# lxd99/TPNet

Hardware: NVIDIA B200
Metric: temporal edges/sec (update+pairwise encode) (higher is better)
Workload: dtype f32

## Files before the change

include/tpnet_b200.h:

```cpp
#ifndef TPNET_B200_H_
#define TPNET_B200_H_

#include <stddef.h>
#include <stdint.h>

#ifdef __cplusplus
extern "C" {
#endif

#define TPN_ABI_VERSION 11

#define TPN_MAX_LAYERS 4

enum {
    TPN_OK = 0,
    TPN_ERR_INVALID_ARGUMENT = -1,
    TPN_ERR_WORKSPACE_TOO_SMALL = -2,
    TPN_ERR_LOG_FULL = -3,
    TPN_ERR_CUDA = -4,
    TPN_ERR_UNSUPPORTED = -5,
    TPN_ERR_INDEX = -6
};

typedef struct tpn_state {
// ... 28 lines not shown
#define TPN_UPDATE_WHOLE 0
#define TPN_UPDATE_PREPARE 1
#define TPN_UPDATE_APPLY 2
int tpn_update_phase(tpn_state_t* st,
                     const int64_t* src_dev, const int64_t* dst_dev, const double* t_dev, int64_t batch,
                     double t_last, float neg_lambda, const float* decay,
                     void* ws_dev, size_t ws_bytes, int32_t* err_flag_dev, void* stream, int phase);

#define TPN_DEBUG_PER_LAYER_WALK 1
#define TPN_DEBUG_SERIAL_WALK 2
#define TPN_DEBUG_SNAPSHOT_P0 4
#define TPN_DEBUG_HEAD_FFMA 8
#define TPN_DEBUG_LEGACY_FRONT 16
#define TPN_DEBUG_NO_STREAM 32
#define TPN_DEBUG_STREAM_ALL 64
int tpn_set_debug_flags(int flags);


int tpn_update_messages(tpn_state_t* st,
                        const int64_t* tgt_dev, const int64_t* src_dev, const double* t_dev, int64_t num_messages,
                        const int32_t* num_messages_dev, int64_t num_local_rows,
                        double t_last, float neg_lambda, const float* decay,
                        void* ws_dev, size_t ws_bytes, int32_t* err_flag_dev, void* stream);

int tpn_gather_blocks(const tpn_state_t* st, const int64_t* ids_dev, int64_t n, float* out_dev, void* stream);

int tpn_pairwise(const tpn_state_t* st, const int64_t* a_ids_dev, const int64_t* b_ids_dev, int64_t n,
                 const int32_t* n_dev, int apply_log_scale, float* out_dev, void* stream);

int tpn_pairwise_neighbors(const tpn_state_t* st, const int64_t* nbr_dev, const int64_t* src_dev,
                           const int64_t* dst_dev, int64_t m, int num_neighbors, int apply_log_scale,
// ... 72 lines not shown
```

tpnet_b200/_lib.py:

```python
from __future__ import annotations

import ctypes
import os
from ctypes import POINTER, c_char_p, c_double, c_float, c_int, c_int32, c_int64, c_size_t, c_void_p
from typing import Optional

_PKG = os.path.dirname(os.path.abspath(__file__))
LIB_PATH = os.path.join(_PKG, '_C', 'libtpnet_b200.so')

TPN_OK = 0
TPN_ERR_LOG_FULL = -3
TPN_ERR_UNSUPPORTED = -5
TPN_ERR_INDEX = -6
STAGE_RAW, STAGE_ID_WRAP, STAGE_ID = 0, 1, 2
TPN_MAX_LAYERS = 4
UPDATE_WHOLE, UPDATE_PREPARE, UPDATE_APPLY = 0, 1, 2
ABI_VERSION = 11

EXPORTED_SYMBOLS = (
    'tpn_version', 'tpn_error_string', 'tpn_last_cuda_error', 'tpn_device_info',
    'tpn_update_workspace_bytes', 'tpn_update', 'tpn_update_phase', 'tpn_pairwise', 'tpn_gather',
    'tpn_materialize', 'tpn_reset_epoch', 'tpn_clear_walk_layers',
    'tpn_stager_create', 'tpn_stager_destroy', 'tpn_stage',
    'tpn_update_messages', 'tpn_gather_blocks', 'tpn_set_debug_flags', 'tpn_pairwise_neighbors', 'tpn_head_forward',
    'tpn_planner_create', 'tpn_planner_destroy', 'tpn_plan', 'tpn_sampler_recent',
    'tpn_route_workspace_bytes', 'tpn_route_update', 'tpn_route_pairs', 'tpn_pull_rows', 'tpn_peer_barrier',
    'tpn_shard_new_generation', 'tpn_peer_alloc', 'tpn_peer_free', 'tpn_ipc_export', 'tpn_ipc_open', 'tpn_ipc_close',
)

SHARD_CTR_NEED, SHARD_CTR_PREV, SHARD_CTR_ERROR, SHARD_COUNTERS = 0, 1, 2, 8


class TpnState(ctypes.Structure):
    _fields_ = [
        ('data', c_void_p),
        ('num_nodes', c_int64),
        ('num_layer', c_int32),
        ('dim', c_int32),
        ('row_stride', c_int64),
# ... 45 lines not shown
    lib.tpn_device_info.restype = c_int
    lib.tpn_device_info.argtypes = [POINTER(c_int), POINTER(c_int), POINTER(c_int)]
    lib.tpn_update_workspace_bytes.restype = c_size_t
    lib.tpn_update_workspace_bytes.argtypes = [POINTER(TpnState), c_int64]
    lib.tpn_update.restype = c_int
    lib.tpn_update.argtypes = [POINTER(TpnState), c_void_p, c_void_p, c_void_p, c_int64, c_double, c_float,
                               POINTER(c_float), c_void_p, c_size_t, c_void_p, c_void_p]
    lib.tpn_update_phase.restype = c_int
    lib.tpn_update_phase.argtypes = [POINTER(TpnState), c_void_p, c_void_p, c_void_p, c_int64, c_double, c_float,
                                     POINTER(c_float), c_void_p, c_size_t, c_void_p, c_void_p, c_int]
    lib.tpn_update_messages.restype = c_int
    lib.tpn_update_messages.argtypes = [POINTER(TpnState), c_void_p, c_void_p, c_void_p, c_int64, c_void_p, c_int64,
                                        c_double, c_float, POINTER(c_float), c_void_p, c_size_t, c_void_p, c_void_p]
    lib.tpn_set_debug_flags.restype = c_int
    lib.tpn_set_debug_flags.argtypes = [c_int]
    lib.tpn_gather_blocks.restype = c_int
    lib.tpn_gather_blocks.argtypes = [POINTER(TpnState), c_void_p, c_int64, c_void_p, c_void_p]
    lib.tpn_pairwise.restype = c_int
    lib.tpn_pairwise.argtypes = [POINTER(TpnState), c_void_p, c_void_p, c_int64, c_void_p, c_int, c_void_p, c_void_p]
    lib.tpn_pairwise_neighbors.restype = c_int
    lib.tpn_pairwise_neighbors.argtypes = [POINTER(TpnState), c_void_p, c_void_p, c_void_p, c_int64, c_int, c_int,
                                           c_void_p, c_void_p]
    lib.tpn_head_forward.restype = c_int
    lib.tpn_head_forward.argtypes = [c_void_p, c_int64, c_void_p, c_int, c_int, c_void_p, c_void_p, c_void_p, c_void_p,
                                     c_void_p, c_void_p]
    lib.tpn_gather.restype = c_int
    lib.tpn_gather.argtypes = [POINTER(TpnState), c_void_p, c_int64, c_void_p, c_void_p]
    for name in ('tpn_materialize', 'tpn_reset_epoch', 'tpn_clear_walk_layers'):
        fn = getattr(lib, name)
        fn.restype = c_int
# ... 77 lines not shown
```

tpnet_b200/csrc/tpn_head_tc.cu:

```cuda
#include <cuda_fp16.h>

#include "tpn_common.cuh"

namespace tpn {

namespace {

constexpr int kF = 64;
constexpr int kHid = 256;
constexpr int kTile = 128;
constexpr int kTcThreads = 160;
constexpr uint32_t kTmemCols = 512;
constexpr uint32_t kD2Col = 256;
constexpr uint32_t kLbo = 128;
constexpr uint32_t kSbo = 1024;
constexpr uint32_t kKStepBytes = 256;

struct TcSmem {
    __half w1[2][kHid * kF];
    __half w2[2][4][kF * 64];
    __half x[2][kTile * kF];
    __half h[2][2][kTile * 64];
    float b1[kHid];
    float b2[kF];
    uint64_t x_full, d1_full, d2_full, h_full[2], h_empty[2];
    uint32_t tmem_base;
    float red[8];
    float w1_inv, w2_inv;
};

__device__ __forceinline__ int canon(int row, int k) { return (row >> 3) * 512 + (k >> 3) * 64 + (row & 7) * 8 + (k & 7); }

__device__ __forceinline__ uint64_t smem_desc(const void* p) {
    const uint32_t addr = smem_u32(p);
    uint64_t d = (uint64_t)((addr & 0x3FFFFu) >> 4);
    d |= (uint64_t)(kLbo >> 4) << 16;
    d |= (uint64_t)(kSbo >> 4) << 32;
    d |= (uint64_t)1 << 46;
    return d;
}

__device__ __forceinline__ constexpr uint32_t instr_desc(int m, int n) {
    return (1u << 4) | ((uint32_t)(n >> 3) << 17) | ((uint32_t)(m >> 4) << 24);
}
// ... 76 lines not shown
                    *reinterpret_cast<uint32_t*>(&l[2]), *reinterpret_cast<uint32_t*>(&l[3]));
}

__device__ __forceinline__ float pow2_scale(float vmax) {
    if (!(vmax > 0.f) || !(vmax < 3.0e38f)) return 1.0f;
    int e;
    (void)frexpf(vmax, &e);
    int s = 14 - e;
    s = s > 100 ? 100 : (s < -100 ? -100 : s);
    return ldexpf(1.0f, s);
}

__global__ void __launch_bounds__(kTcThreads, 1)
head_tc_kernel(const float* __restrict__ x, long long n, const float* __restrict__ w1, const float* __restrict__ b1,
               const float* __restrict__ w2, const float* __restrict__ b2, float* __restrict__ y,
               const int* __restrict__ n_dev) {
    if (n_dev != nullptr) n = min(n, (long long)max(*n_dev, 0));
    extern __shared__ __align__(128) unsigned char tc_raw[];
    TcSmem& sm = *reinterpret_cast<TcSmem*>(tc_raw);
    const int tid = threadIdx.x, warp = tid >> 5, lane = tid & 31;
    const long long ntiles = (n + kTile - 1) / kTile;

    if (tid == 0) {
        mbar_init(&sm.x_full, kTile);
        mbar_init(&sm.d1_full, 1);
        mbar_init(&sm.d2_full, 1);
        for (int i = 0; i < 2; ++i) {
            mbar_init(&sm.h_full[i], kTile);
            mbar_init(&sm.h_empty[i], 1);
        }
        asm volatile("fence.mbarrier_init.release.cluster;" ::: "memory");
// ... 58 lines not shown
    tc_fence_after();
    const uint32_t tmem = sm.tmem_base;
    const float w1_inv = sm.w1_inv, w2_inv = sm.w2_inv;

    uint32_t it = 0;
    if (warp < 4) {
        const int r = tid;
        const uint32_t lane_base = (uint32_t)(warp * 32) << 16;
        float4 xn[kF / 4];
        auto load_x = [&](long long tile) {
            const long long row = tile * kTile + r;
            const bool ok = tile < ntiles && row < n;
#pragma unroll
            for (int q = 0; q < kF / 4; ++q) xn[q] = ok ? ld4(x + row * kF + 4 * q) : make_float4(0.f, 0.f, 0.f, 0.f);
        };
        auto split_x = [&]() -> float {
            float vmax = 0.f;
#pragma unroll
            for (int q = 0; q < kF / 4; ++q)
                vmax = fmaxf(vmax, fmaxf(fmaxf(fabsf(xn[q].x), fabsf(xn[q].y)), fmaxf(fabsf(xn[q].z), fabsf(xn[q].w))));
            const float sx = pow2_scale(vmax);
#pragma unroll
            for (int k8 = 0; k8 < kF / 8; ++k8) {
                const float4 a = xn[2 * k8], b = xn[2 * k8 + 1];
                const float v[8] = {a.x * sx, a.y * sx, a.z * sx, a.w * sx, b.x * sx, b.y * sx, b.z * sx, b.w * sx};
                uint4 hi, lo;
                split8(v, hi, lo);
                *reinterpret_cast<uint4*>(&sm.x[0][canon(r, k8 * 8)]) = hi;
                *reinterpret_cast<uint4*>(&sm.x[1][canon(r, k8 * 8)]) = lo;
            }
            fence_proxy_async_smem();
            tc_fence_before();
            mbar_arrive(&sm.x_full);
            return w1_inv / sx;
        };
        long long tile = blockIdx.x;
        load_x(tile);
        float inv1 = split_x();
        load_x(tile + gridDim.x);
        for (; tile < ntiles; tile += gridDim.x, ++it) {
            const long long row = tile * kTile + r;
            const bool valid = row < n;
            mbar_wait_bounded(&sm.d1_full, it & 1u);
            tc_fence_after();
            float inv2[4];
#pragma unroll 1
            for (int c = 0; c < 4; ++c) {
                const int buf = c & 1;
                const uint32_t use = it * 2u + (uint32_t)(c >> 1);
                float d0[32], d1[32];
                tmem_ld32_nowait(tmem + lane_base + (uint32_t)(c * 64), d0);
                tmem_ld32_nowait(tmem + lane_base + (uint32_t)(c * 64 + 32), d1);
                tmem_ld_wait();
                float hmax = 0.f;
#pragma unroll
// ... 7 lines not shown
                mbar_wait_bounded(&sm.h_empty[buf], (use & 1u) ^ 1u);
#pragma unroll
                for (int k8 = 0; k8 < 8; ++k8) {
                    float v[8];
#pragma unroll
                    for (int j = 0; j < 8; ++j) v[j] = (k8 < 4 ? d0[k8 * 8 + j] : d1[(k8 - 4) * 8 + j]) * sh;
                    uint4 hi, lo;
                    split8(v, hi, lo);
                    *reinterpret_cast<uint4*>(&sm.h[buf][0][canon(r, k8 * 8)]) = hi;
                    *reinterpret_cast<uint4*>(&sm.h[buf][1][canon(r, k8 * 8)]) = lo;
                }
                fence_proxy_async_smem();
                mbar_arrive(&sm.h_full[buf]);
            }
            const float inv2_0 = inv2[0], inv2_1 = inv2[1], inv2_2 = inv2[2], inv2_3 = inv2[3];
            if (tile + gridDim.x < ntiles) {
                inv1 = split_x();
                load_x(tile + 2 * (long long)gridDim.x);
            }
            mbar_wait_bounded(&sm.d2_full, it & 1u);
            tc_fence_after();
#pragma unroll 1
            for (int half = 0; half < 2; ++half) {
                float d[32];
                {
                    float d1[32], d2[32], d3[32];
                    tmem_ld32_nowait(tmem + lane_base + kD2Col + (uint32_t)(half * 32), d);
                    tmem_ld32_nowait(tmem + lane_base + kD2Col + 64u + (uint32_t)(half * 32), d1);
                    tmem_ld32_nowait(tmem + lane_base + kD2Col + 128u + (uint32_t)(half * 32), d2);
                    tmem_ld32_nowait(tmem + lane_base + kD2Col + 192u + (uint32_t)(half * 32), d3);
                    tmem_ld_wait();
#pragma unroll
                    for (int j = 0; j < 32; ++j)
                        d[j] = (d[j] * inv2_0 + d1[j] * inv2_1) + (d2[j] * inv2_2 + d3[j] * inv2_3);
                }
                if (valid) {
#pragma unroll
                    for (int q = 0; q < 8; ++q) {
                        const int o = half * 32 + q * 4;
                        st4(y + row * kF + o, make_float4(d[q * 4] + sm.b2[o], d[q * 4 + 1] + sm.b2[o + 1],
                                                          d[q * 4 + 2] + sm.b2[o + 2], d[q * 4 + 3] + sm.b2[o + 3]));
                    }
                }
            }
            tc_fence_before();
        }
    } else if (lane == 0) {
        constexpr uint32_t idesc1 = instr_desc(kTile, kHid), idesc2 = instr_desc(kTile, kF);
        const uint64_t xa[2] = {smem_desc(sm.x[0]), smem_desc(sm.x[1])};
        const uint64_t wb[2] = {smem_desc(sm.w1[0]), smem_desc(sm.w1[1])};
        auto gemm1 = [&](uint32_t t) {
            mbar_wait_bounded(&sm.x_full, t & 1u);
            tc_fence_after();
#pragma unroll
            for (int ks = 0; ks < kF / 16; ++ks) {
                const uint64_t adv = (uint64_t)((ks * kKStepBytes) >> 4);
                mma_f16(tmem, xa[0] + adv, wb[1] + adv, idesc1, ks > 0 ? 1u : 0u);
                mma_f16(tmem, xa[1] + adv, wb[0] + adv, idesc1, 1u);
            }
#pragma unroll
            for (int ks = 0; ks < kF / 16; ++ks) {
                const uint64_t adv = (uint64_t)((ks * kKStepBytes) >> 4);
                mma_f16(tmem, xa[0] + adv, wb[0] + adv, idesc1, 1u);
            }
            mma_commit(&sm.d1_full);
        };
        long long tile = blockIdx.x;
        if (tile < ntiles) gemm1(0);
        for (; tile < ntiles; tile += gridDim.x, ++it) {
#pragma unroll 1
            for (int c = 0; c < 4; ++c) {
                const int buf = c & 1;
                const uint32_t use = it * 2u + (uint32_t)(c >> 1);
                mbar_wait_bounded(&sm.h_full[buf], use & 1u);
                tc_fence_after();
                const uint64_t ha[2] = {smem_desc(sm.h[buf][0]), smem_desc(sm.h[buf][1])};
                const uint64_t vb[2] = {smem_desc(sm.w2[0][c]), smem_desc(sm.w2[1][c])};
                const uint32_t dacc = tmem + kD2Col + (uint32_t)(c * 64);
#pragma unroll
                for (int ks = 0; ks < 4; ++ks) {
                    const uint64_t adv = (uint64_t)((ks * kKStepBytes) >> 4);
                    mma_f16(dacc, ha[0] + adv, vb[1] + adv, idesc2, ks > 0 ? 1u : 0u);
                    mma_f16(dacc, ha[1] + adv, vb[0] + adv, idesc2, 1u);
                }
#pragma unroll
                for (int ks = 0; ks < 4; ++ks) {
                    const uint64_t adv = (uint64_t)((ks * kKStepBytes) >> 4);
                    mma_f16(dacc, ha[0] + adv, vb[0] + adv, idesc2, 1u);
                }
                mma_commit(&sm.h_empty[buf]);
            }
            mma_commit(&sm.d2_full);
            if (tile + gridDim.x < ntiles) gemm1(it + 1u);
        }
    }

    tc_fence_before();
    __syncthreads();
    if (warp == 4) {
        asm volatile("tcgen05.dealloc.cta_group::1.sync.aligned.b32 %0, %1;" ::"r"(tmem), "r"(kTmemCols) : "memory");
    }
}

}

int launch_head_tensor(const float* x, long long n, const int* n_dev, const float* w1, const float* b1, const float* w2,
                       const float* b2, float* y, int dev_slot, cudaStream_t stream) {
    static bool configured_tab[kMaxDevices];
    bool& configured = configured_tab[dev_slot];
    const int smem = (int)sizeof(TcSmem);
    if (!configured) {
        const cudaError_t e = cudaFuncSetAttribute(head_tc_kernel, cudaFuncAttributeMaxDynamicSharedMemorySize, smem);
        if (e != cudaSuccess) {
            set_cuda_error(e);
            return TPN_ERR_CUDA;
        }
        configured = true;
    }
    const long long ntiles = (n + kTile - 1) / kTile;
    const int sms = device_sm_count();
    const unsigned grid = (unsigned)(ntiles < sms ? ntiles : sms);
    head_tc_kernel<<<grid, kTcThreads, smem, stream>>>(x, n, w1, b1, w2, b2, y, n_dev);
    return TPN_OK;
}

}
```

tpnet_b200/csrc/tpn_update.cu:

```cuda
#include <stdlib.h>

#include "tpn_common.cuh"

namespace tpn {

namespace {

int g_debug_flags = 0;
thread_local int g_dev_slot = 0;

constexpr int kSmallMaxMsgs = 4096;
constexpr int kRankMaxMsgs = 1024;
constexpr int kPrepThreads = 1024;
constexpr int kRadixThreads = 256;
constexpr int kRadixItems = 8;
constexpr int kRadixTile = kRadixThreads * kRadixItems;
constexpr int kRadixBins = 256;
constexpr int kRadixDirectBlocks = 16;
constexpr int kWalkThreads = 256;
constexpr int kHubMin = 64;
constexpr int kGiantMin = 2048;
constexpr int kHubConsumers = 4;
constexpr int kHubThreads = (kHubConsumers + 1) * 32;
constexpr int kHubStages = 4;
// ... 8 lines not shown
#ifndef TPN_HUB2_GIANT_FLOATS
#define TPN_HUB2_GIANT_FLOATS 16
#endif
constexpr int kHub2GiantFloats = TPN_HUB2_GIANT_FLOATS;
static_assert(kHub2GiantFloats == 8 || kHub2GiantFloats == 16 || kHub2GiantFloats == 32, "giant slices are 32, 64 or 128 bytes");
constexpr int kGiantLs = kHub2GiantFloats == 8 ? 1 : (kHub2GiantFloats == 16 ? 2 : 3);
constexpr int kGiantSpm = 16 >> kGiantLs;
constexpr int kGiantSpmMax = kGiantSpm > 4 ? kGiantSpm : 4;
constexpr int kHub2Stages = kHub2Producers + 4;
constexpr int kCtrGiant = 0, kCtrHub = 1, kCtrWork0 = 2, kCtrSmall = 6, kCtrHub2Work = 7, kCtrHub2Giant = 8;
constexpr int kCtrChunks = 9;
constexpr int kCtrStream = 10, kCtrStreamBlocks = 11, kCtrStreamProd = 12, kCtrStreamActive = 13, kCtrStreamChain = 14, kCtrStreamTicket = 15;
constexpr int kStreamSlice = kHub2GiantFloats;
constexpr int kStreamBlock = 32 * kGiantSpm;
constexpr uint32_t kNoPart = 0xffffffffu;
constexpr int kCtrSmClaim = 16;
constexpr int kCtrSlots = kCtrSmClaim + 256;
constexpr int kBarWords = 32;

struct DecayArgs {
    float c[TPN_MAX_LAYERS];
    int has_decay;
};

struct Count {
    int cap;
    const int* dev;
    __device__ __forceinline__ int get() const {
        if (dev == nullptr) return cap;
        const int v = *dev;
        return v < 0 ? 0 : (v > cap ? cap : v);
// ... 36 lines not shown
    uint32_t* sslot;
    uint32_t* slen;
    float* snap;
    uint32_t* hub_giant;
    uint32_t* hub_reg;
    uint32_t* ctr;
    uint32_t* small_heads;
    uint32_t* hub_len;
    uint32_t* hub_part;
    uint32_t* giant_cbase;
    float* partial;
    int* svst;
    float* gprod;
    uint32_t* gflag;
    uint32_t* gblk;
    bool has_snap;
    bool has_stream;
    size_t bytes;
};

inline size_t snap_bytes(size_t E, int num_layer, int64_t row_stride) {
    return sizeof(float) * E * (size_t)num_layer * (size_t)row_stride;
}

inline size_t align_up(size_t x, size_t a) { return (x + a - 1) / a * a; }

constexpr size_t kStreamMaxBytes = (size_t)4 << 30;
constexpr int kGiantSortMaxC = 2048;
inline int stream_slices(int num_layer, int64_t row_stride) {
    return num_layer * (int)((row_stride + kStreamSlice - 1) / kStreamSlice);
// ... 28 lines not shown
    const size_t hub_cap = E / kHubMin + E / kChunkMin + E / kGiantMin + 4;
    const size_t part_rows = E / kChunkMin + E / kGiantMin + 2;
    ws.hub_reg = reinterpret_cast<uint32_t*>(take(4 * hub_cap));
    ws.hub_len = reinterpret_cast<uint32_t*>(take(4 * hub_cap));
    ws.hub_part = reinterpret_cast<uint32_t*>(take(4 * hub_cap));
    ws.giant_cbase = reinterpret_cast<uint32_t*>(take(4 * (E / kGiantMin + 2)));
    ws.partial = reinterpret_cast<float*>(take(ws.has_snap ? 4 * part_rows * (size_t)num_layer * (size_t)row_stride : 16));
    ws.ctr = reinterpret_cast<uint32_t*>(take(4 * kCtrSlots));
    ws.small_heads = reinterpret_cast<uint32_t*>(take(4 * E));
    ws.svst = reinterpret_cast<int*>(take(4 * (E + 4) * (size_t)(num_layer > 1 ? num_layer - 1 : 1) + 16));
    ws.gflag = reinterpret_cast<uint32_t*>(take(4 * stream_flag_words(E)));
    ws.gblk = reinterpret_cast<uint32_t*>(take(4 * (kGiantSortMaxC + 1)));
    ws.has_stream = ws.has_snap && stream_prod_bytes(E, num_layer, row_stride) <= kStreamMaxBytes &&
                    E / kGiantMin + 2 <= (size_t)kGiantSortMaxC;
    ws.gprod = reinterpret_cast<float*>(take(ws.has_stream ? stream_prod_bytes(E, num_layer, row_stride) : 16));
    ws.bytes = off;
    return ws;
}

__device__ __forceinline__ float edge_weight(double t, float t_last_f, float neg_lambda) {
    const float diff = __fsub_rn(t_last_f, (float)t);
    const float arg = __fmul_rn(neg_lambda, diff);
    return (float)exp((double)arg);
}

struct SweepArgs {
    long long total4;
    int ds4;
};

// ... 460 lines not shown
        if (small_head) small_heads[base + __popc(mask & ((1u << lane) - 1u))] = (uint32_t)p;
    }
}

__global__ void __launch_bounds__(256) payload_kernel(PayloadArgs a) {
    payload_body(a, blockIdx.x * blockDim.x + threadIdx.x);
}

constexpr int kGiantSortMax = kGiantSortMaxC;
struct GiantSmem {
    uint32_t head_s[kGiantSortMax], len_s[kGiantSortMax], sorted_s[kGiantSortMax];
};
__device__ __forceinline__ void sort_giants_body(GiantSmem& sm, uint32_t* __restrict__ hub_giant,
                                                 const uint32_t* __restrict__ slen, uint32_t* __restrict__ ctr,
                                                 uint32_t* __restrict__ gblk, uint32_t* __restrict__ gflag, Count count,
                                                 int stream_mode) {
    const uint32_t stream_min = stream_mode == 0 ? 0u
                                : (stream_mode == 2 ? (uint32_t)kGiantMin
                                                    : max((uint32_t)kGiantMin, (uint32_t)(count.get() >> 2)));
    const int n = (int)ctr[kCtrGiant];
    if (n < 1 || n > kGiantSortMax) return;
    for (int i = threadIdx.x; i < n; i += blockDim.x) {
        sm.head_s[i] = hub_giant[i];
        sm.len_s[i] = slen[sm.head_s[i]];
    }
    __syncthreads();
    for (int i = threadIdx.x; i < n; i += blockDim.x) {
        const uint32_t li = sm.len_s[i];
        int rank = 0;
        for (int j = 0; j < n; ++j) rank += (sm.len_s[j] > li || (sm.len_s[j] == li && j < i)) ? 1 : 0;
        hub_giant[rank] = sm.head_s[i];
        sm.sorted_s[rank] = li;
    }
    __syncthreads();
    if (threadIdx.x == 0 && stream_min > 0) {
        uint32_t blocks = 0;
        int ns = 0;
        for (; ns < n && sm.sorted_s[ns] >= stream_min; ++ns) {
            gblk[ns] = blocks;
            blocks += (sm.sorted_s[ns] + (uint32_t)kStreamBlock - 1u) / (uint32_t)kStreamBlock;
        }
        gblk[ns] = blocks;
        ctr[kCtrStream] = (uint32_t)ns;
        ctr[kCtrStreamBlocks] = blocks;
        sm.head_s[0] = blocks;
    }
    __syncthreads();
    if (stream_min > 0) {
        const uint32_t blocks = sm.head_s[0];
        for (uint32_t i = threadIdx.x; i < blocks; i += blockDim.x) gflag[i] = 0;
    }
}
__global__ void __launch_bounds__(1024)
sort_giants_kernel(uint32_t* __restrict__ hub_giant, const uint32_t* __restrict__ slen, uint32_t* __restrict__ ctr,
                   uint32_t* __restrict__ gblk, uint32_t* __restrict__ gflag, Count count, int stream_mode) {
    __shared__ GiantSmem sm;
    sort_giants_body(sm, hub_giant, slen, ctr, gblk, gflag, count, stream_mode);
}

struct FrontArgs {
    PrepArgs prep;
    uint32_t *key_a, *key_b, *val_a, *val_b, *hist, *hist2, *bar;
    int passes;
};

__device__ __forceinline__ void grid_barrier(uint32_t* bar, uint32_t& target, int* err_flag) {
    __syncthreads();
    if (threadIdx.x == 0) {
        target += gridDim.x;
        __threadfence();
        atomicAdd(bar, 1u);
        uint32_t seen;
// ... 892 lines not shown
    }
}

__host__ __device__ inline size_t hub2_smem_bytes() {
    return (size_t)kHub2Stages * (32 * kHub2SlotFloats * 4 + 16) + 16;
}

template <bool LAZY, bool DIRECT>
__global__ void __launch_bounds__(kHub2Threads, 2)
walk_hub2_kernel(StateView st, const uint32_t* __restrict__ skey, const uint32_t* __restrict__ ssrc,
                 const float* __restrict__ sw, const uint32_t* __restrict__ sslot,
                 const uint32_t* __restrict__ slen, const float* __restrict__ snap,
                 const uint32_t* __restrict__ hub_giant, const uint32_t* __restrict__ hub_reg,
                 uint32_t* __restrict__ ctr, int spr_g, int slice_w_g, int spr_r, int slice_w_r, DecayArgs dnow,
                 const uint32_t* __restrict__ hub_len, const uint32_t* __restrict__ hub_part,
                 float* __restrict__ partial, int chunked, int srow0) {
    extern __shared__ __align__(128) unsigned char hub2_raw[];
    float* const ring = reinterpret_cast<float*>(hub2_raw);
    uint64_t* const full = reinterpret_cast<uint64_t*>(ring + (size_t)kHub2Stages * 32 * kHub2SlotFloats);
    uint64_t* const empty = full + kHub2Stages;
    int* const item = reinterpret_cast<int*>(empty + kHub2Stages);
    const int warp = threadIdx.x >> 5;
    const int lane = threadIdx.x & 31;
    const int L = st.num_layer;
    const int rs = (int)st.row_stride;
    if (threadIdx.x == 0) {
        for (int i = 0; i < kHub2Stages; ++i) {
            mbar_init(&full[i], 32);
            mbar_init(&empty[i], 1);
        }
        asm volatile("fence.mbarrier_init.release.cluster;" ::: "memory");
        unsigned smid;
        asm volatile("mov.u32 %0, %%smid;" : "=r"(smid));
        *item = (smid < 256u && atomicAdd(&ctr[kCtrSmClaim + smid], 1u) == 0u) ? 1 : 0;
    }
    __syncthreads();
    const bool prefer_giant = *item != 0;
    __syncthreads();
    const uint32_t n_stream = ctr[kCtrStream];
    const uint32_t n_giant = ctr[kCtrGiant] - n_stream, n_reg = ctr[kCtrHub];
    const uint32_t slices_g = (uint32_t)(L * spr_g), slices_r = (uint32_t)(L * spr_r);
    const uint32_t total_g = chunked ? 0u : n_giant * slices_g, total_r = n_reg * slices_r;
    uint32_t blk_base = 0;
    for (;;) {
        if (threadIdx.x == 0) {
            int w = -1;
            if (prefer_giant && total_g > 0) {
                const uint32_t g = atomicAdd(&ctr[kCtrHub2Giant], 1u);
                if (g < total_g) w = (int)g;
            }
            if (w == -1 && total_r > 0) {
                const uint32_t q = atomicAdd(&ctr[kCtrHub2Work], 1u);
                if (q < total_r) w = -(int)q - 2;
            }
            *item = w;
        }
        __syncthreads();
        const int work = *item;
        __syncthreads();
        if (work == -1) break;
        const bool giant = work >= 0;
        const uint32_t idx = giant ? (uint32_t)work : (uint32_t)(-(work + 2));
        const int spr = giant ? spr_g : spr_r;
        const int slice_w = giant ? slice_w_g : slice_w_r;
        const uint32_t slices = giant ? slices_g : slices_r;
        const uint32_t hub_i = idx / slices;
        const int slice = (int)(idx - hub_i * slices);
        const uint32_t hub = giant ? hub_i + n_stream : hub_i;
        const int r = slice / spr;
        const int c0 = (slice - r * spr) * slice_w;
        const int width = min(rs, c0 + slice_w) - c0;
        const int head = (int)(giant ? hub_giant[hub] : hub_reg[hub]);
        const int len = (int)(giant ? slen[head] : hub_len[hub]);
        const uint32_t part = giant ? kNoPart : hub_part[hub];
        const uint32_t key = skey[head];
        const int spm = giant ? kGiantSpm : 1;
        const int slot = giant ? kHub2GiantFloats : kHub2SlotFloats;
        const int mps = 32 * spm;
        const int nblk = (len + mps - 1) / mps;
        if (width > 0) {
            if (warp >= 1) {
                const int pw = warp - 1;
                const int nvec = width >> 2;
// ... 114 lines not shown
                                acc.y = __fadd_rn(acc.y, p.y);
                            }
                        }
                        for (; j0 < nm; ++j0) {
                            const float2 p = *reinterpret_cast<const float2*>(xs + j0 * kHub2SlotFloats);
                            acc.x = __fadd_rn(acc.x, p.x);
                            acc.y = __fadd_rn(acc.y, p.y);
                        }
                    }
                    HUB2_STAMP(b, 2);
                    __syncwarp();
                    if (lane == 0) mbar_arrive(&empty[stage]);
                    HUB2_STAMP(b, 3);
                }
                if (active) {
                    if (giant) *tptr = acc.x;
                    else *reinterpret_cast<float2*>(tptr) = acc;
                }
            }
        }
        blk_base += (width > 0) ? (uint32_t)nblk : 0u;
    }
}

template <bool LAZY>
__global__ void __launch_bounds__(256)
combine_giants_kernel(StateView st, const uint32_t* __restrict__ skey, const uint32_t* __restrict__ slen,
                      const uint32_t* __restrict__ hub_giant, const uint32_t* __restrict__ giant_cbase,
                      const uint32_t* __restrict__ ctr, const float* __restrict__ partial, int chunk) {
    const int L = st.num_layer;
    const int rs = (int)st.row_stride;
// ... 15 lines not shown
            uint32_t c = 0;
            for (; c + 4 <= nch; c += 4) {
                const float p0 = pbase[(long long)(c + 0) * span + col], p1 = pbase[(long long)(c + 1) * span + col];
                const float p2 = pbase[(long long)(c + 2) * span + col], p3 = pbase[(long long)(c + 3) * span + col];
                acc = __fadd_rn(__fadd_rn(__fadd_rn(__fadd_rn(acc, p0), p1), p2), p3);
            }
            for (; c < nch; ++c) acc = __fadd_rn(acc, pbase[(long long)c * span + col]);
            trow[col] = acc;
        }
    }
}


template <bool DIRECT>
int launch_walk_hub2(const StateView& v, const Workspace& ws, bool lazy, const DecayArgs& dnow, int chunk, int srow0,
                     cudaStream_t stream) {
    static bool configured_tab[kMaxDevices];
    bool& configured = configured_tab[g_dev_slot];
    const int smem = (int)hub2_smem_bytes();
    if (!configured) {
        cudaError_t e = cudaFuncSetAttribute(walk_hub2_kernel<false, DIRECT>, cudaFuncAttributeMaxDynamicSharedMemorySize, smem);
        if (e == cudaSuccess)
            e = cudaFuncSetAttribute(walk_hub2_kernel<true, DIRECT>, cudaFuncAttributeMaxDynamicSharedMemorySize, smem);
        if (e != cudaSuccess) {
            set_cuda_error(e);
            return TPN_ERR_CUDA;
        }
        configured = true;
    }
    const int rs = (int)v.row_stride;
    const int spr_r = (rs + kHub2SlotFloats - 1) / kHub2SlotFloats;
    const int slice_w_r = (((rs + spr_r - 1) / spr_r) + 3) & ~3;
    const int spr_g = (rs + kHub2GiantFloats - 1) / kHub2GiantFloats;
    const int slice_w_g = (((rs + spr_g - 1) / spr_g) + 3) & ~3;
    const unsigned grid = (unsigned)device_sm_count() * 2;
    const int chunked = chunk > 0 ? 1 : 0;
    if (lazy)
        walk_hub2_kernel<true, DIRECT><<<grid, kHub2Threads, smem, stream>>>(v, ws.key_a, ws.ssrc, ws.sw, ws.sslot, ws.slen,
                                                                             ws.snap, ws.hub_giant, ws.hub_reg, ws.ctr,
                                                                             spr_g, slice_w_g, spr_r, slice_w_r, dnow,
                                                                             ws.hub_len, ws.hub_part, ws.partial, chunked,
                                                                             srow0);
    else
        walk_hub2_kernel<false, DIRECT><<<grid, kHub2Threads, smem, stream>>>(v, ws.key_a, ws.ssrc, ws.sw, ws.sslot, ws.slen,
                                                                              ws.snap, ws.hub_giant, ws.hub_reg, ws.ctr,
                                                                              spr_g, slice_w_g, spr_r, slice_w_r, dnow,
                                                                              ws.hub_len, ws.hub_part, ws.partial, chunked,
                                                                              srow0);
    if (chunked) {
        const unsigned cgrid = (unsigned)device_sm_count();
        if (lazy)
            combine_giants_kernel<true><<<cgrid, 256, 0, stream>>>(v, ws.key_a, ws.slen, ws.hub_giant, ws.giant_cbase,
                                                                   ws.ctr, ws.partial, chunk);
        else
            combine_giants_kernel<false><<<cgrid, 256, 0, stream>>>(v, ws.key_a, ws.slen, ws.hub_giant, ws.giant_cbase,
                                                                    ws.ctr, ws.partial, chunk);
    }
    return TPN_OK;
}

template <bool DIRECT>
int launch_walk_stream(const StateView& v, const Workspace& ws, bool lazy, int srow0, int* err_flag_dev, cudaStream_t stream) {
    static bool configured_tab[kMaxDevices];
// ... 185 lines not shown
    const float t_last_f = (float)t_last;
    double* log_w = lazy ? st->decay_log : nullptr;
    const bool force_per_layer = (g_debug_flags & TPN_DEBUG_PER_LAYER_WALK) != 0;
    const bool snapshot_path = ws.has_snap && !(force_per_layer && !(count_dev == nullptr && E <= kSmallMaxMsgs));
    const bool small_path = count_dev == nullptr && E <= kSmallMaxMsgs;
    const bool hubs = !small_path;
    const int E4 = (E + 3) & ~3;
    const bool eager_sweep = !lazy && dargs.has_decay;
    int chunk = st->giant_chunk > 0 ? (int)st->giant_chunk : 0;
    if (chunk > 0 && chunk < kChunkMin) chunk = kChunkMin;
    if (chunk > kGiantMin) chunk = kGiantMin;
    chunk &= ~31;
    const long long sweep_total4 = st->num_nodes * (long long)L * ds4;
    const int stream_mode = (ws.has_stream && chunk == 0 && (g_debug_flags & TPN_DEBUG_NO_STREAM) == 0)
                                ? ((g_debug_flags & TPN_DEBUG_STREAM_ALL) ? 2 : 1) : 0;

    StateView view = make_view(st);
    view.epoch = new_epoch;

    const bool do_front = phase != TPN_UPDATE_APPLY;
    const bool do_rest = phase != TPN_UPDATE_PREPARE;
    const bool snap_early = lazy && !small_path;
    if (small_path) {
        if (phase == TPN_UPDATE_PREPARE) return TPN_OK;
        SweepArgs sw_args;
        sw_args.total4 = eager_sweep ? sweep_total4 : 0;
        sw_args.ds4 = ds4;
        unsigned grid = 1;
        if (eager_sweep) {
            const long long want = (sweep_total4 + kPrepThreads - 1) / kPrepThreads;
// ... 56 lines not shown
            fr.passes = passes;
            const int sms = device_sm_count();
            const unsigned grid = (unsigned)(nblk < 1 ? 1 : (nblk < sms ? nblk : sms));
            void* kargs[] = {&fr};
            if (cudaMemsetAsync(ws.bar, 0, 4 * kBarWords, stream) != cudaSuccess ||
                cudaLaunchCooperativeKernel((const void*)front_kernel, dim3(grid), dim3(kRadixThreads), kargs, 0,
                                            stream) != cudaSuccess) {
                set_cuda_error(cudaGetLastError());
                return TPN_ERR_CUDA;
            }
            const bool odd = (passes & 1) != 0;
            fa.pay.order = odd ? ws.val_b : ws.val_a;
            fa.pay.skey = odd ? ws.key_b : ws.key_a;
            payload_kernel<<<(E + 255) / 256, 256, 0, stream>>>(fa.pay);
            if (snapshot_path && chunk == 0) {
                sort_giants_kernel<<<1, 1024, 0, stream>>>(ws.hub_giant, ws.slen, ws.ctr, ws.gblk, ws.gflag, cnt, stream_mode);
            }
        } else
        {
            prep_large_kernel<<<(unsigned)((E + 255) / 256 < 2 ? 2 : (E + 255) / 256), 256, 0, stream>>>(fa.prep);
            uint32_t *kin = ws.key_a, *kout = ws.key_b, *vin = ws.val_a, *vout = ws.val_b;
            for (int p = 0; p < passes; ++p) {
                radix_hist_kernel<<<nblk, kRadixThreads, 0, stream>>>(kin, cnt, 8 * p, ws.hist);
                const int prefixed = (nblk > kRadixDirectBlocks || count_dev != nullptr) ? 1 : 0;
                if (prefixed) radix_prefix_kernel<<<kRadixBins / 8, 256, 0, stream>>>(ws.hist, cnt);
                radix_scatter_kernel<<<nblk, kRadixThreads, 0, stream>>>(kin, vin, kout, vout, cnt, 8 * p, ws.hist,
                                                                         prefixed);
                uint32_t* tk = kin; kin = kout; kout = tk;
                uint32_t* tv = vin; vin = vout; vout = tv;
            }
            fa.pay.order = vin;
            fa.pay.skey = kin;
            payload_kernel<<<(E + 255) / 256, 256, 0, stream>>>(fa.pay);
            if (snapshot_path && chunk == 0) {
                sort_giants_kernel<<<1, 1024, 0, stream>>>(ws.hub_giant, ws.slen, ws.ctr, ws.gblk, ws.gflag, cnt, stream_mode);
            }
        }
    }
    if (!small_path && do_rest && eager_sweep) {
        const long long want = (sweep_total4 + 255) / 256;
        const long long cap = (long long)device_sm_count() * 16;
        const unsigned grid = (unsigned)(want < cap ? (want < 1 ? 1 : want) : cap);
        sweep_decay_kernel<<<grid, 256, 0, stream>>>(view, dargs, sweep_total4, ds4);
    }

    const int srow0 = (g_debug_flags & TPN_DEBUG_SNAPSHOT_P0) ? 0 : 1;
    if (snapshot_path) {
        if (L - srow0 >= 1 && (snap_early ? do_front : do_rest)) {
            const unsigned grid = (unsigned)(((long long)E * 32 + 255) / 256);
            if (lazy) snapshot_kernel<true><<<grid, 256, 0, stream>>>(view, ws.key_a, cnt, ds4, ws.snap, srow0);
            else snapshot_kernel<false><<<grid, 256, 0, stream>>>(view, ws.key_a, cnt, ds4, ws.snap, srow0);
        }
        if (!do_rest) {
        } else if (hubs) {
            const bool direct = msgs.B == 0;
            SideStream* side = (g_debug_flags & TPN_DEBUG_SERIAL_WALK) ? nullptr : side_stream();
            cudaStream_t hub_stream = stream, giant_stream = stream;
            if (side != nullptr) {
                if (cudaEventRecord(side->fork, stream) == cudaSuccess &&
                    cudaStreamWaitEvent(side->stream, side->fork, 0) == cudaSuccess) {
                    hub_stream = side->stream;
                    if (stream_mode > 0 && cudaStreamWaitEvent(side->stream2, side->fork, 0) == cudaSuccess)
                        giant_stream = side->stream2;
                } else {
                    (void)cudaGetLastError();
                }
            }
            if (stream_mode > 0) {
// ... 60 lines not shown
    const size_t have = sizeof(tpn::g_hub2_timeline) / sizeof(unsigned long long);
    if (host_out == nullptr || count > have) return TPN_ERR_INVALID_ARGUMENT;
    return cudaMemcpyFromSymbol(host_out, tpn::g_hub2_timeline, count * sizeof(unsigned long long)) == cudaSuccess
               ? TPN_OK : TPN_ERR_CUDA;
}
#endif

namespace tpn {
int debug_flags() { return g_debug_flags; }
}

extern "C" int tpn_set_debug_flags(int flags) {
    const int old = tpn::g_debug_flags;
    tpn::g_debug_flags = flags;
    return old;
}

extern "C" int tpn_update(tpn_state_t* st, const int64_t* src_dev, const int64_t* dst_dev, const double* t_dev,
                          int64_t batch, double t_last, float neg_lambda, const float* decay, void* ws_dev,
                          size_t ws_bytes, int32_t* err_flag_dev, void* stream_v) {
    using namespace tpn;
    int rc = validate_state(st);
    if (rc != TPN_OK) return rc;
    if (batch < 1 || batch > ((int64_t)1 << 26) || src_dev == nullptr || dst_dev == nullptr || t_dev == nullptr ||
        ws_dev == nullptr || st->num_nodes >= (int64_t)0xffffffffll)
        return TPN_ERR_INVALID_ARGUMENT;
    DeviceScope scope(st->data);
    g_dev_slot = scope.slot();
    MsgSource msgs;
    msgs.a = reinterpret_cast<const long long*>(src_dev);
// ... 52 lines not shown
```

Before: 155.0 million.

## Precompute largest giant hubs during prepare phase; dynamic tile claiming in head kernel

During the PREPARE phase, up to two of the largest giant hubs are walked early into a workspace buffer. The APPLY phase then copies those results into state and skips them in the giant work queue, moving long-tail work earlier so it can overlap with other stages. Separately, the tensor-core head kernel now hands out tiles through a global atomic counter with per-launch claim slots instead of a fixed grid stride, for better load balance. This adds a workspace buffer, extra atomics and barriers, and a debug query function.

```diff
diff --git a/include/tpnet_b200.h b/include/tpnet_b200.h
--- a/include/tpnet_b200.h
+++ b/include/tpnet_b200.h
@@ -66,7 +66,9 @@
 #define TPN_DEBUG_LEGACY_FRONT 16
 #define TPN_DEBUG_NO_STREAM 32
 #define TPN_DEBUG_STREAM_ALL 64
+#define TPN_DEBUG_NO_EARLY_GIANTS 128
 int tpn_set_debug_flags(int flags);
+int tpn_debug_early_giants(const tpn_state_t* st, int64_t batch, const void* ws_dev, int32_t* count_out);
 
 
 int tpn_update_messages(tpn_state_t* st,
diff --git a/tpnet_b200/_lib.py b/tpnet_b200/_lib.py
--- a/tpnet_b200/_lib.py
+++ b/tpnet_b200/_lib.py
@@ -22,7 +22,7 @@
     'tpn_update_workspace_bytes', 'tpn_update', 'tpn_update_phase', 'tpn_pairwise', 'tpn_gather',
     'tpn_materialize', 'tpn_reset_epoch', 'tpn_clear_walk_layers',
     'tpn_stager_create', 'tpn_stager_destroy', 'tpn_stage',
-    'tpn_update_messages', 'tpn_gather_blocks', 'tpn_set_debug_flags', 'tpn_pairwise_neighbors', 'tpn_head_forward',
+    'tpn_update_messages', 'tpn_gather_blocks', 'tpn_set_debug_flags', 'tpn_debug_early_giants', 'tpn_pairwise_neighbors', 'tpn_head_forward',
     'tpn_planner_create', 'tpn_planner_destroy', 'tpn_plan', 'tpn_sampler_recent',
     'tpn_route_workspace_bytes', 'tpn_route_update', 'tpn_route_pairs', 'tpn_pull_rows', 'tpn_peer_barrier',
     'tpn_shard_new_generation', 'tpn_peer_alloc', 'tpn_peer_free', 'tpn_ipc_export', 'tpn_ipc_open', 'tpn_ipc_close',
@@ -98,6 +98,8 @@
                                         c_double, c_float, POINTER(c_float), c_void_p, c_size_t, c_void_p, c_void_p]
     lib.tpn_set_debug_flags.restype = c_int
     lib.tpn_set_debug_flags.argtypes = [c_int]
+    lib.tpn_debug_early_giants.restype = c_int
+    lib.tpn_debug_early_giants.argtypes = [POINTER(TpnState), c_int64, c_void_p, POINTER(c_int32)]
     lib.tpn_gather_blocks.restype = c_int
     lib.tpn_gather_blocks.argtypes = [POINTER(TpnState), c_void_p, c_int64, c_void_p, c_void_p]
     lib.tpn_pairwise.restype = c_int
diff --git a/tpnet_b200/csrc/tpn_head_tc.cu b/tpnet_b200/csrc/tpn_head_tc.cu
--- a/tpnet_b200/csrc/tpn_head_tc.cu
+++ b/tpnet_b200/csrc/tpn_head_tc.cu
@@ -24,10 +24,20 @@
     float b1[kHid];
     float b2[kF];
     uint64_t x_full, d1_full, d2_full, h_full[2], h_empty[2];
+    long long claimed;
+    uint32_t x_valid;
     uint32_t tmem_base;
     float red[8];
     float w1_inv, w2_inv;
 };
+
+constexpr int kClaimSlots = 256;
+struct TileClaim {
+    unsigned long long next;
+    unsigned int done;
+    unsigned int pad;
+};
+__device__ TileClaim g_head_claim[kClaimSlots];
 
 __device__ __forceinline__ int canon(int row, int k) { return (row >> 3) * 512 + (k >> 3) * 64 + (row & 7) * 8 + (k & 7); }
 
@@ -134,7 +144,7 @@
 __global__ void __launch_bounds__(kTcThreads, 1)
 head_tc_kernel(const float* __restrict__ x, long long n, const float* __restrict__ w1, const float* __restrict__ b1,
                const float* __restrict__ w2, const float* __restrict__ b2, float* __restrict__ y,
-               const int* __restrict__ n_dev) {
+               const int* __restrict__ n_dev, int claim_slot) {
     if (n_dev != nullptr) n = min(n, (long long)max(*n_dev, 0));
     extern __shared__ __align__(128) unsigned char tc_raw[];
     TcSmem& sm = *reinterpret_cast<TcSmem*>(tc_raw);
@@ -223,7 +233,20 @@
 #pragma unroll
             for (int q = 0; q < kF / 4; ++q) xn[q] = ok ? ld4(x + row * kF + 4 * q) : make_float4(0.f, 0.f, 0.f, 0.f);
         };
-        auto split_x = [&]() -> float {
+        TileClaim& claim = g_head_claim[claim_slot];
+        auto next_tile = [&]() -> long long {
+            if (tid == 0) sm.claimed = (long long)gridDim.x + (long long)atomicAdd(&claim.next, 1ull);
+            asm volatile("bar.sync 1, %0;" ::"n"(kTile) : "memory");
+            const long long t = sm.claimed;
+            asm volatile("bar.sync 1, %0;" ::"n"(kTile) : "memory");
+            return t;
+        };
+        auto split_x = [&](bool valid) -> float {
+            if (r == 0) sm.x_valid = valid ? 1u : 0u;
+            if (!valid) {
+                mbar_arrive(&sm.x_full);
+                return 0.f;
+            }
             float vmax = 0.f;
 #pragma unroll
             for (int q = 0; q < kF / 4; ++q)
@@ -245,9 +268,10 @@
         };
         long long tile = blockIdx.x;
         load_x(tile);
-        float inv1 = split_x();
-        load_x(tile + gridDim.x);
-        for (; tile < ntiles; tile += gridDim.x, ++it) {
+        float inv1 = split_x(tile < ntiles);
+        long long next = tile < ntiles ? next_tile() : ntiles;
+        load_x(next);
+        for (; tile < ntiles; ++it) {
             const long long row = tile * kTile + r;
             const bool valid = row < n;
             mbar_wait_bounded(&sm.d1_full, it & 1u);
@@ -285,9 +309,11 @@
                 mbar_arrive(&sm.h_full[buf]);
             }
             const float inv2_0 = inv2[0], inv2_1 = inv2[1], inv2_2 = inv2[2], inv2_3 = inv2[3];
-            if (tile + gridDim.x < ntiles) {
-                inv1 = split_x();
-                load_x(tile + 2 * (long long)gridDim.x);
+            inv1 = split_x(next < ntiles);
+            long long after = ntiles;
+            if (next < ntiles) {
+                after = next_tile();
+                load_x(after);
             }
             mbar_wait_bounded(&sm.d2_full, it & 1u);
             tc_fence_after();
@@ -315,14 +341,17 @@
                 }
             }
             tc_fence_before();
+            tile = next;
+            next = after;
         }
     } else if (lane == 0) {
         constexpr uint32_t idesc1 = instr_desc(kTile, kHid), idesc2 = instr_desc(kTile, kF);
         const uint64_t xa[2] = {smem_desc(sm.x[0]), smem_desc(sm.x[1])};
         const uint64_t wb[2] = {smem_desc(sm.w1[0]), smem_desc(sm.w1[1])};
-        auto gemm1 = [&](uint32_t t) {
+        auto gemm1 = [&](uint32_t t) -> bool {
             mbar_wait_bounded(&sm.x_full, t & 1u);
             tc_fence_after();
+            if (sm.x_valid == 0u) return false;
 #pragma unroll
             for (int ks = 0; ks < kF / 16; ++ks) {
                 const uint64_t adv = (uint64_t)((ks * kKStepBytes) >> 4);
@@ -335,10 +364,9 @@
                 mma_f16(tmem, xa[0] + adv, wb[0] + adv, idesc1, 1u);
             }
             mma_commit(&sm.d1_full);
+            return true;
         };
-        long long tile = blockIdx.x;
-        if (tile < ntiles) gemm1(0);
-        for (; tile < ntiles; tile += gridDim.x, ++it) {
+        for (bool more = gemm1(0); more; ++it) {
 #pragma unroll 1
             for (int c = 0; c < 4; ++c) {
                 const int buf = c & 1;
@@ -362,7 +390,7 @@
                 mma_commit(&sm.h_empty[buf]);
             }
             mma_commit(&sm.d2_full);
-            if (tile + gridDim.x < ntiles) gemm1(it + 1u);
+            more = gemm1(it + 1u);
         }
     }
 
@@ -370,6 +398,13 @@
     __syncthreads();
     if (warp == 4) {
         asm volatile("tcgen05.dealloc.cta_group::1.sync.aligned.b32 %0, %1;" ::"r"(tmem), "r"(kTmemCols) : "memory");
+    }
+    if (tid == 0) {
+        TileClaim& claim = g_head_claim[claim_slot];
+        if (atomicAdd(&claim.done, 1u) == gridDim.x - 1u) {
+            claim.next = 0ull;
+            claim.done = 0u;
+        }
     }
 }
 
@@ -391,7 +426,9 @@
     const long long ntiles = (n + kTile - 1) / kTile;
     const int sms = device_sm_count();
     const unsigned grid = (unsigned)(ntiles < sms ? ntiles : sms);
-    head_tc_kernel<<<grid, kTcThreads, smem, stream>>>(x, n, w1, b1, w2, b2, y, n_dev);
+    static unsigned next_slot[kMaxDevices];
+    const int slot = (int)(next_slot[dev_slot]++ % (unsigned)kClaimSlots);
+    head_tc_kernel<<<grid, kTcThreads, smem, stream>>>(x, n, w1, b1, w2, b2, y, n_dev, slot);
     return TPN_OK;
 }
 
diff --git a/tpnet_b200/csrc/tpn_update.cu b/tpnet_b200/csrc/tpn_update.cu
--- a/tpnet_b200/csrc/tpn_update.cu
+++ b/tpnet_b200/csrc/tpn_update.cu
@@ -46,7 +46,10 @@
 constexpr int kStreamSlice = kHub2GiantFloats;
 constexpr int kStreamBlock = 32 * kGiantSpm;
 constexpr uint32_t kNoPart = 0xffffffffu;
-constexpr int kCtrSmClaim = 16;
+constexpr int kCtrEarly = 16, kCtrEarlyWork = 17;
+constexpr int kEarlyMax = 2;
+constexpr int kEarlyShift = 4;
+constexpr int kCtrSmClaim = 18;
 constexpr int kCtrSlots = kCtrSmClaim + 256;
 constexpr int kBarWords = 32;
 
@@ -113,6 +116,7 @@
     float* gprod;
     uint32_t* gflag;
     uint32_t* gblk;
+    float* early;
     bool has_snap;
     bool has_stream;
     size_t bytes;
@@ -171,6 +175,7 @@
     ws.has_stream = ws.has_snap && stream_prod_bytes(E, num_layer, row_stride) <= kStreamMaxBytes &&
                     E / kGiantMin + 2 <= (size_t)kGiantSortMaxC;
     ws.gprod = reinterpret_cast<float*>(take(ws.has_stream ? stream_prod_bytes(E, num_layer, row_stride) : 16));
+    ws.early = reinterpret_cast<float*>(take(sizeof(float) * kEarlyMax * (size_t)num_layer * (size_t)row_stride));
     ws.bytes = off;
     return ws;
 }
@@ -661,10 +666,11 @@
 __device__ __forceinline__ void sort_giants_body(GiantSmem& sm, uint32_t* __restrict__ hub_giant,
                                                  const uint32_t* __restrict__ slen, uint32_t* __restrict__ ctr,
                                                  uint32_t* __restrict__ gblk, uint32_t* __restrict__ gflag, Count count,
-                                                 int stream_mode) {
+                                                 int stream_mode, int early_max) {
     const uint32_t stream_min = stream_mode == 0 ? 0u
                                 : (stream_mode == 2 ? (uint32_t)kGiantMin
                                                     : max((uint32_t)kGiantMin, (uint32_t)(count.get() >> 2)));
+    const uint32_t early_min = max((uint32_t)kGiantMin, (uint32_t)(count.get() >> kEarlyShift));
     const int n = (int)ctr[kCtrGiant];
     if (n < 1 || n > kGiantSortMax) return;
     for (int i = threadIdx.x; i < n; i += blockDim.x) {
@@ -680,17 +686,22 @@
         sm.sorted_s[rank] = li;
     }
     __syncthreads();
-    if (threadIdx.x == 0 && stream_min > 0) {
-        uint32_t blocks = 0;
+    if (threadIdx.x == 0) {
         int ns = 0;
-        for (; ns < n && sm.sorted_s[ns] >= stream_min; ++ns) {
+        if (stream_min > 0) {
+            uint32_t blocks = 0;
+            for (; ns < n && sm.sorted_s[ns] >= stream_min; ++ns) {
+                gblk[ns] = blocks;
+                blocks += (sm.sorted_s[ns] + (uint32_t)kStreamBlock - 1u) / (uint32_t)kStreamBlock;
+            }
             gblk[ns] = blocks;
-            blocks += (sm.sorted_s[ns] + (uint32_t)kStreamBlock - 1u) / (uint32_t)kStreamBlock;
-        }
-        gblk[ns] = blocks;
-        ctr[kCtrStream] = (uint32_t)ns;
-        ctr[kCtrStreamBlocks] = blocks;
-        sm.head_s[0] = blocks;
+            ctr[kCtrStream] = (uint32_t)ns;
+            ctr[kCtrStreamBlocks] = blocks;
+            sm.head_s[0] = blocks;
+        }
+        int ne = 0;
+        while (ne < early_max && ns + ne < n && sm.sorted_s[ns + ne] >= early_min) ++ne;
+        ctr[kCtrEarly] = (uint32_t)ne;
     }
     __syncthreads();
     if (stream_min > 0) {
@@ -700,9 +711,10 @@
 }
 __global__ void __launch_bounds__(1024)
 sort_giants_kernel(uint32_t* __restrict__ hub_giant, const uint32_t* __restrict__ slen, uint32_t* __restrict__ ctr,
-                   uint32_t* __restrict__ gblk, uint32_t* __restrict__ gflag, Count count, int stream_mode) {
+                   uint32_t* __restrict__ gblk, uint32_t* __restrict__ gflag, Count count, int stream_mode,
+                   int early_max) {
     __shared__ GiantSmem sm;
-    sort_giants_body(sm, hub_giant, slen, ctr, gblk, gflag, count, stream_mode);
+    sort_giants_body(sm, hub_giant, slen, ctr, gblk, gflag, count, stream_mode, early_max);
 }
 
 struct FrontArgs {
@@ -1625,7 +1637,7 @@
                  const uint32_t* __restrict__ hub_giant, const uint32_t* __restrict__ hub_reg,
                  uint32_t* __restrict__ ctr, int spr_g, int slice_w_g, int spr_r, int slice_w_r, DecayArgs dnow,
                  const uint32_t* __restrict__ hub_len, const uint32_t* __restrict__ hub_part,
-                 float* __restrict__ partial, int chunked, int srow0) {
+                 float* __restrict__ partial, int chunked, int srow0, float* __restrict__ early, int early_mode) {
     extern __shared__ __align__(128) unsigned char hub2_raw[];
     float* const ring = reinterpret_cast<float*>(hub2_raw);
     uint64_t* const full = reinterpret_cast<uint64_t*>(ring + (size_t)kHub2Stages * 32 * kHub2SlotFloats);
@@ -1643,21 +1655,30 @@
         asm volatile("fence.mbarrier_init.release.cluster;" ::: "memory");
         unsigned smid;
         asm volatile("mov.u32 %0, %%smid;" : "=r"(smid));
-        *item = (smid < 256u && atomicAdd(&ctr[kCtrSmClaim + smid], 1u) == 0u) ? 1 : 0;
+        *item = early_mode || (smid < 256u && atomicAdd(&ctr[kCtrSmClaim + smid], 1u) == 0u) ? 1 : 0;
     }
     __syncthreads();
     const bool prefer_giant = *item != 0;
     __syncthreads();
     const uint32_t n_stream = ctr[kCtrStream];
-    const uint32_t n_giant = ctr[kCtrGiant] - n_stream, n_reg = ctr[kCtrHub];
+    const uint32_t n_early = ctr[kCtrEarly];
+    const uint32_t g_first = n_stream + (early_mode ? 0u : n_early);
+    const uint32_t n_giant = early_mode ? n_early : ctr[kCtrGiant] - g_first;
+    const uint32_t n_reg = early_mode ? 0u : ctr[kCtrHub];
     const uint32_t slices_g = (uint32_t)(L * spr_g), slices_r = (uint32_t)(L * spr_r);
+    if (!early_mode && blockIdx.x < n_early) {
+        const uint32_t key = skey[hub_giant[n_stream + blockIdx.x]];
+        const float4* src = reinterpret_cast<const float4*>(early + (size_t)blockIdx.x * L * rs);
+        float4* dst = reinterpret_cast<float4*>(st.data + (long long)key * st.node_stride + rs);
+        for (int i = threadIdx.x; i < (L * rs) >> 2; i += kHub2Threads) dst[i] = src[i];
+    }
     const uint32_t total_g = chunked ? 0u : n_giant * slices_g, total_r = n_reg * slices_r;
     uint32_t blk_base = 0;
     for (;;) {
         if (threadIdx.x == 0) {
             int w = -1;
             if (prefer_giant && total_g > 0) {
-                const uint32_t g = atomicAdd(&ctr[kCtrHub2Giant], 1u);
+                const uint32_t g = atomicAdd(&ctr[early_mode ? kCtrEarlyWork : kCtrHub2Giant], 1u);
                 if (g < total_g) w = (int)g;
             }
             if (w == -1 && total_r > 0) {
@@ -1677,7 +1698,7 @@
         const uint32_t slices = giant ? slices_g : slices_r;
         const uint32_t hub_i = idx / slices;
         const int slice = (int)(idx - hub_i * slices);
-        const uint32_t hub = giant ? hub_i + n_stream : hub_i;
+        const uint32_t hub = giant ? hub_i + g_first : hub_i;
         const int r = slice / spr;
         const int c0 = (slice - r * spr) * slice_w;
         const int width = min(rs, c0 + slice_w) - c0;
@@ -1822,7 +1843,8 @@
                     HUB2_STAMP(b, 3);
                 }
                 if (active) {
-                    if (giant) *tptr = acc.x;
+                    if (early_mode) early[((size_t)hub_i * L + r) * rs + c0 + col] = acc.x;
+                    else if (giant) *tptr = acc.x;
                     else *reinterpret_cast<float2*>(tptr) = acc;
                 }
             }
@@ -1868,7 +1890,7 @@
 
 template <bool DIRECT>
 int launch_walk_hub2(const StateView& v, const Workspace& ws, bool lazy, const DecayArgs& dnow, int chunk, int srow0,
-                     cudaStream_t stream) {
+                     cudaStream_t stream, int early_mode = 0) {
     static bool configured_tab[kMaxDevices];
     bool& configured = configured_tab[g_dev_slot];
     const int smem = (int)hub2_smem_bytes();
@@ -1887,20 +1909,22 @@
     const int slice_w_r = (((rs + spr_r - 1) / spr_r) + 3) & ~3;
     const int spr_g = (rs + kHub2GiantFloats - 1) / kHub2GiantFloats;
     const int slice_w_g = (((rs + spr_g - 1) / spr_g) + 3) & ~3;
-    const unsigned grid = (unsigned)device_sm_count() * 2;
+    const int sms = device_sm_count();
+    const int early_items = kEarlyMax * v.num_layer * spr_g;
+    const unsigned grid = early_mode ? (unsigned)(early_items < sms ? early_items : sms) : (unsigned)sms * 2;
     const int chunked = chunk > 0 ? 1 : 0;
     if (lazy)
         walk_hub2_kernel<true, DIRECT><<<grid, kHub2Threads, smem, stream>>>(v, ws.key_a, ws.ssrc, ws.sw, ws.sslot, ws.slen,
                                                                              ws.snap, ws.hub_giant, ws.hub_reg, ws.ctr,
                                                                              spr_g, slice_w_g, spr_r, slice_w_r, dnow,
                                                                              ws.hub_len, ws.hub_part, ws.partial, chunked,
-                                                                             srow0);
+                                                                             srow0, ws.early, early_mode);
     else
         walk_hub2_kernel<false, DIRECT><<<grid, kHub2Threads, smem, stream>>>(v, ws.key_a, ws.ssrc, ws.sw, ws.sslot, ws.slen,
                                                                               ws.snap, ws.hub_giant, ws.hub_reg, ws.ctr,
                                                                               spr_g, slice_w_g, spr_r, slice_w_r, dnow,
                                                                               ws.hub_len, ws.hub_part, ws.partial, chunked,
-                                                                              srow0);
+                                                                              srow0, ws.early, early_mode);
     if (chunked) {
         const unsigned cgrid = (unsigned)device_sm_count();
         if (lazy)
@@ -2116,6 +2140,8 @@
     const long long sweep_total4 = st->num_nodes * (long long)L * ds4;
     const int stream_mode = (ws.has_stream && chunk == 0 && (g_debug_flags & TPN_DEBUG_NO_STREAM) == 0)
                                 ? ((g_debug_flags & TPN_DEBUG_STREAM_ALL) ? 2 : 1) : 0;
+    const bool early_giants = phase == TPN_UPDATE_PREPARE && lazy && snapshot_path && !small_path && chunk == 0 &&
+                              msgs.B > 0 && count_dev == nullptr && (g_debug_flags & TPN_DEBUG_NO_EARLY_GIANTS) == 0;
 
     StateView view = make_view(st);
     view.epoch = new_epoch;
@@ -2202,7 +2228,8 @@
             fa.pay.skey = odd ? ws.key_b : ws.key_a;
             payload_kernel<<<(E + 255) / 256, 256, 0, stream>>>(fa.pay);
             if (snapshot_path && chunk == 0) {
-                sort_giants_kernel<<<1, 1024, 0, stream>>>(ws.hub_giant, ws.slen, ws.ctr, ws.gblk, ws.gflag, cnt, stream_mode);
+                sort_giants_kernel<<<1, 1024, 0, stream>>>(ws.hub_giant, ws.slen, ws.ctr, ws.gblk, ws.gflag, cnt, stream_mode,
+                                                           early_giants ? kEarlyMax : 0);
             }
         } else
         {
@@ -2221,7 +2248,8 @@
             fa.pay.skey = kin;
             payload_kernel<<<(E + 255) / 256, 256, 0, stream>>>(fa.pay);
             if (snapshot_path && chunk == 0) {
-                sort_giants_kernel<<<1, 1024, 0, stream>>>(ws.hub_giant, ws.slen, ws.ctr, ws.gblk, ws.gflag, cnt, stream_mode);
+                sort_giants_kernel<<<1, 1024, 0, stream>>>(ws.hub_giant, ws.slen, ws.ctr, ws.gblk, ws.gflag, cnt, stream_mode,
+                                                           early_giants ? kEarlyMax : 0);
             }
         }
     }
@@ -2240,6 +2268,10 @@
             else snapshot_kernel<false><<<grid, 256, 0, stream>>>(view, ws.key_a, cnt, ds4, ws.snap, srow0);
         }
         if (!do_rest) {
+            if (early_giants) {
+                const int erc = launch_walk_hub2<false>(view, ws, lazy, dargs, chunk, srow0, stream, 1);
+                if (erc != TPN_OK) return erc;
+            }
         } else if (hubs) {
             const bool direct = msgs.B == 0;
             SideStream* side = (g_debug_flags & TPN_DEBUG_SERIAL_WALK) ? nullptr : side_stream();
@@ -2330,6 +2362,20 @@
     const int old = tpn::g_debug_flags;
     tpn::g_debug_flags = flags;
     return old;
+}
+
+extern "C" int tpn_debug_early_giants(const tpn_state_t* st, int64_t batch, const void* ws_dev, int32_t* count_out) {
+    using namespace tpn;
+    if (st == nullptr || ws_dev == nullptr || count_out == nullptr || batch < 1) return TPN_ERR_INVALID_ARGUMENT;
+    DeviceScope scope(st->data);
+    const Workspace ws = carve(const_cast<void*>(ws_dev), batch, st->num_layer, st->row_stride);
+    uint32_t n = 0;
+    if (cudaDeviceSynchronize() != cudaSuccess || cudaMemcpy(&n, ws.ctr + kCtrEarly, 4, cudaMemcpyDeviceToHost) != cudaSuccess) {
+        set_cuda_error(cudaGetLastError());
+        return TPN_ERR_CUDA;
+    }
+    *count_out = (int32_t)n;
+    return TPN_OK;
 }
 
 extern "C" int tpn_update(tpn_state_t* st, const int64_t* src_dev, const int64_t* dst_dev, const double* t_dev,
```

After: 156.7 million (median of 6 runs). 1.1% higher.
